# 0x09/dspfun

Measured on AMD Instinct MI355X. Metric: Mpixels/s DCT-II+III roundtrip 3840x2160x3, higher is better.
Workload: dtype f32

## Files before the change

### dspfun_amd/_lib.py

```python
import ctypes as C
import os

_HERE = os.path.dirname(os.path.abspath(__file__))
LIB_PATH = os.environ.get("DSPFFT_LIB_PATH") or os.path.join(_HERE, "csrc", "libdspfft_hip.so")

REDFT01, REDFT10 = 4, 5

SYMBOLS = [
    "dspfft_plan_many_r2r", "dspfft_plan_r2r_2d", "dspfft_plan_set_scale", "dspfft_plan_set_axis_scale0",
    "dspfft_plan_many_r2r_f64", "dspfft_plan_set_scale_f64", "dspfft_plan_set_axis_scale0_f64", "dspfft_execute_f64", "dspfft_execute_masked_accumulate_f64", "dspfft_plan_scan_prepare", "dspfft_plan_set_input_window", "dspfft_plan_set_output_alternate", "dspfft_set_plan_effort", "dspfft_get_plan_effort",
    "dspfft_plan_many_r2r_ordered", "dspfft_plan_guru_r2r", "dspfft_execute_roundtrip", "dspfft_execute_roundtrip_u8", "dspfft_execute_roundtrip_u8_dither",
    "dspfft_roundtrip_topn_work_bytes", "dspfft_execute_roundtrip_topn", "dspfft_execute_roundtrip_u8_topn", "dspfft_motion_topn_blocks_work_bytes", "dspfft_motion_topn_blocks",
    "dspfft_execute", "dspfft_plan_num_passes", "dspfft_execute_pass", "dspfft_destroy_plan", "dspfft_plan_describe", "dspfft_plan_algorithmic_bytes",
    "dspfft_execute_many", "dspfft_execute_many_repeat", "dspfft_execute_sum2", "dspfft_cosrows_create", "dspfft_cosrows_execute", "dspfft_cosrows_destroy", "dspfft_cztrows_create", "dspfft_cztrows_execute", "dspfft_cztrows_execute_n", "dspfft_cztrows_length", "dspfft_cztrows_destroy", "dspfft_transpose_f32", "dspfft_plan_set_input_modulation", "dspfft_stream_create", "dspfft_stream_destroy", "dspfft_stream_synchronize", "dspfft_event_create", "dspfft_event_destroy", "dspfft_event_synchronize", "dspfft_event_elapsed_ms",
    "dspfft_last_error", "dspfft_version", "dspfft_set_thread_plan_effort", "dspfft_get_thread_plan_effort", "dspfft_fftw_sparse_uploads",
    "dspfft_scan_zigzag", "dspfft_scan_zigzag_frame_ids", "dspfft_execute_masked_accumulate", "dspfft_execute_masked_accumulate_range", "dspfft_execute_masked_accumulate_range_f64", "dspfft_scan_scatter", "dspfft_accumulate", "dspfft_broadcast_dc",
    "dspfft_scan_limit", "dspfft_scan_max_interval", "dspfft_scan_coord_slots", "dspfft_scan_owner_index", "dspfft_scan_frame_ids", "dspfft_scan_coords", "dspfft_scan_stamp",
    "dspfft_scan_index_to_frame_ids", "dspfft_scan_magnitude_work_bytes", "dspfft_scan_magnitude_index",
    "dspfft_u8_to_f32", "dspfft_f32_to_u8",
    "dspfft_zoom_ncomponents", "dspfft_zoom_basis", "dspfft_zoom_work_floats", "dspfft_zoom_product", "dspfft_gemm_nt_f32",
    "dspfft_zoom_last_error", "dspfft_zoomfft_create", "dspfft_zoomfft_work_floats", "dspfft_zoomfft_execute", "dspfft_zoomfft_destroy", "dspfft_zoomfft_last_error", "dspfft_zoomczt_create", "dspfft_zoomczt_work_floats", "dspfft_zoomczt_execute", "dspfft_zoomczt_destroy",
    "dspfft_zoomanim_create", "dspfft_zoomanim_work_floats", "dspfft_zoomanim_set_coeffs", "dspfft_zoomanim_execute", "dspfft_zoomanim_destroy", "dspfft_zoomanim_last_error",
    "dspfft_scanframes_create", "dspfft_scanframes_frame_floats", "dspfft_scanframes_begin", "dspfft_scanframes_mark_range", "dspfft_scanframes_mark_coords",
    "dspfft_scanframes_compose", "dspfft_scanframes_parity", "dspfft_scanframes_destroy",
    "dspfft_trc_from_name", "dspfft_trc_name", "dspfft_trc_apply_f32", "dspfft_scanframes_set_trc", "dspfft_zoomanim_set_trc",
    "dspfft_motion_load_f32_linear", "dspfft_motion_store_f32_linear",
    "dspfft_plan_set_u8_trc", "dspfft_u8_to_f32_trc", "dspfft_f32_to_u8_trc", "dspfft_motion_load_u8_linear", "dspfft_motion_store_u8_linear", "dspfft_motion_dither_u8_trc",
    "dspfft_applybasis_work_floats", "dspfft_applybasis_partsums",
    "dspfft_applybasis_work_floats_ex", "dspfft_applybasis_partsums_ex", "dspfft_applybasis_render",
    "dspfft_motion_load_u8", "dspfft_motion_store_u8", "dspfft_motion_load_f32", "dspfft_motion_store_f32", "dspfft_motion_topn_work_bytes", "dspfft_motion_topn", "dspfft_motion_last_error", "dspfft_motion_dither_u8",
    "dspfft_spec_encode", "dspfft_ispec_decode", "dspfft_ispec_signmap", "dspfft_motion_filter", "dspfft_scan_pruned_accumulate", "dspfft_scan_pruned_work_floats", "dspfft_scan_pruned_accumulate_ws", "dspfft_pointwise_last_error",
]

class IoDim(C.Structure):
    _fields_ = [("n", C.c_int), ("is_", C.c_int), ("os", C.c_int)]


class DitherGeom(C.Structure):
    _fields_ = [("n", C.c_int * 3), ("row_pitch", C.c_longlong), ("plane_pitch", C.c_longlong), ("nblocks", C.c_int * 3), ("block_step", C.c_longlong * 3)]


class ScanFrameOpts(C.Structure):
    _fields_ = [("visualize", C.c_int), ("spectrogram", C.c_int), ("intermediates", C.c_int), ("max_intermediates", C.c_int),
                ("spec_gain", C.c_double), ("spec_scaletype", C.c_int), ("spec_signtype", C.c_int), ("parity_depth", C.c_int)]


class MotionFilterParams(C.Structure):
    _fields_ = [("active", C.c_int * 3), ("minbuf_hw", C.c_int * 2), ("block_depth", C.c_int), ("band_begin", C.c_int * 3), ("band_end", C.c_int * 3),
                ("damp", C.c_float), ("boost", C.c_float), ("threshold_lo", C.c_float), ("threshold_hi", C.c_float),
                ("preserve_dc", C.c_int), ("grey_add", C.c_float), ("quantizer", C.c_float)]


_lib = None


def bind(lib):
    ip = C.POINTER(C.c_int)
    vp = C.c_void_p
    lib.dspfft_plan_many_r2r.argtypes = [C.POINTER(vp), C.c_int, ip, C.c_int, ip, C.c_int, C.c_int, ip, C.c_int, C.c_int, ip]
    lib.dspfft_plan_r2r_2d.argtypes = [C.POINTER(vp), C.c_int, C.c_int, C.c_int, C.c_int]
    lib.dspfft_plan_set_scale.argtypes = [vp, C.c_float]
    lib.dspfft_plan_set_axis_scale0.argtypes = [vp, C.c_int, C.c_float, C.c_float]
    lib.dspfft_execute.argtypes = [vp, vp, vp, vp]
    lib.dspfft_execute_sum2.argtypes = [vp, vp, vp, vp, vp, vp]
    lib.dspfft_cosrows_create.argtypes = [C.POINTER(vp), C.c_int, C.c_int, C.c_int, C.c_int]
    lib.dspfft_cosrows_execute.argtypes = [vp, vp, C.c_longlong, vp, C.c_longlong, C.c_double, C.c_double, vp]
    lib.dspfft_cosrows_destroy.argtypes = [vp]
    lib.dspfft_cosrows_destroy.restype = None
    lib.dspfft_cztrows_create.argtypes = [C.POINTER(vp), C.c_int, C.c_int, C.c_int, C.c_int]
    lib.dspfft_cztrows_execute.argtypes = [vp, vp, C.c_longlong, C.c_longlong, C.c_int, vp, C.c_longlong, C.c_longlong, C.c_int, C.c_double, C.c_double, C.c_double, vp]
    lib.dspfft_cztrows_execute_n.argtypes = [vp, C.c_int, C.c_int, vp, C.c_longlong, C.c_longlong, C.c_int, vp, C.c_longlong, C.c_longlong, C.c_int, C.c_double, C.c_double, C.c_double, vp]
    lib.dspfft_zoomanim_create.argtypes = [C.POINTER(vp), C.c_int, C.c_int, C.c_int, C.c_int, C.c_int]
    lib.dspfft_zoomanim_work_floats.restype = C.c_size_t
    lib.dspfft_zoomanim_work_floats.argtypes = [vp]
    lib.dspfft_zoomanim_set_coeffs.argtypes = [vp, vp, vp]
    lib.dspfft_zoomanim_execute.argtypes = [vp] + [C.c_double] * 6 + [C.c_int, C.c_int, vp, vp, vp]
    lib.dspfft_zoomanim_destroy.argtypes = [vp]
    lib.dspfft_zoomanim_destroy.restype = None
    lib.dspfft_zoomanim_last_error.restype = C.c_char_p
    lib.dspfft_cztrows_length.argtypes = [vp]
    lib.dspfft_cztrows_destroy.argtypes = [vp]
    lib.dspfft_cztrows_destroy.restype = None
    lib.dspfft_transpose_f32.argtypes = [vp, C.c_longlong, vp, C.c_longlong, C.c_int, C.c_int, vp]
    lib.dspfft_plan_set_input_modulation.argtypes = [vp, C.c_int, vp, C.c_int]
    lib.dspfft_plan_set_input_window.argtypes = [vp, C.c_int, C.c_int, C.c_int]
    lib.dspfft_plan_set_output_alternate.argtypes = [vp, C.c_int, C.c_int]
    lib.dspfft_execute_many.argtypes = [C.c_int, C.POINTER(vp), C.POINTER(vp), C.POINTER(vp), C.POINTER(vp), C.c_int, C.c_int, C.POINTER(vp)]
    lib.dspfft_execute_many_repeat.argtypes = [C.c_int, C.POINTER(vp), C.POINTER(vp), C.POINTER(vp), C.POINTER(vp), C.c_int, C.c_int, C.c_int, C.c_int, C.POINTER(vp)]
    lib.dspfft_stream_create.restype = vp
    lib.dspfft_stream_create.argtypes = []
    lib.dspfft_stream_destroy.argtypes = [vp]
    lib.dspfft_stream_synchronize.argtypes = [vp]
    lib.dspfft_event_create.restype = vp
    lib.dspfft_event_create.argtypes = []
    lib.dspfft_event_destroy.argtypes = [vp]
    lib.dspfft_event_destroy.restype = None
    lib.dspfft_event_synchronize.argtypes = [vp]
    lib.dspfft_event_elapsed_ms.argtypes = [vp, vp, C.POINTER(C.c_float)]
    lib.dspfft_plan_many_r2r_f64.argtypes = lib.dspfft_plan_many_r2r.argtypes
    lib.dspfft_plan_many_r2r_ordered.argtypes = lib.dspfft_plan_many_r2r.argtypes + [C.c_int]
    lib.dspfft_plan_guru_r2r.argtypes = [C.POINTER(vp), C.c_int, C.POINTER(IoDim), C.c_int, C.POINTER(IoDim), ip, C.c_int]
    lib.dspfft_execute_roundtrip.argtypes = [vp, vp, vp, vp, C.POINTER(MotionFilterParams), vp, vp]
    lib.dspfft_execute_roundtrip_u8.argtypes = [vp, vp, vp, vp, vp, C.c_double, C.POINTER(MotionFilterParams), vp, vp]
    lib.dspfft_execute_roundtrip_u8_dither.argtypes = [vp, vp, vp, vp, vp, C.c_double, C.c_double, C.POINTER(MotionFilterParams), vp, vp]
    if hasattr(lib, "dspfft_execute_roundtrip_topn"):
        lib.dspfft_roundtrip_topn_work_bytes.restype = C.c_size_t
        lib.dspfft_roundtrip_topn_work_bytes.argtypes = [vp, vp]
        lib.dspfft_execute_roundtrip_topn.argtypes = [vp, vp, vp, vp, C.POINTER(MotionFilterParams), C.c_size_t, vp, C.c_size_t, vp, vp]
        lib.dspfft_execute_roundtrip_u8_topn.argtypes = [vp, vp, vp, vp, vp, C.c_double, C.POINTER(MotionFilterParams), C.c_size_t, vp, C.c_size_t, vp, vp]
    lib.dspfft_plan_set_scale_f64.argtypes = [vp, C.c_double]
    lib.dspfft_plan_set_axis_scale0_f64.argtypes = [vp, C.c_int, C.c_double, C.c_double]
    lib.dspfft_execute_f64.argtypes = [vp, vp, vp, vp]
    lib.dspfft_execute_masked_accumulate_f64.argtypes = [vp, vp, vp, vp, vp, C.c_uint32, C.c_int, vp]
    lib.dspfft_plan_scan_prepare.argtypes = [vp, vp, C.c_int, vp]
    lib.dspfft_set_plan_effort.argtypes = [C.c_int]
    lib.dspfft_set_plan_effort.restype = None
    lib.dspfft_get_plan_effort.argtypes = []
    lib.dspfft_plan_num_passes.argtypes = [vp]
    lib.dspfft_execute_pass.argtypes = [vp, C.c_int, vp, vp, vp]
    lib.dspfft_destroy_plan.argtypes = [vp]
    lib.dspfft_destroy_plan.restype = None
    lib.dspfft_plan_describe.argtypes = [vp, C.c_char_p, C.c_size_t]
    lib.dspfft_plan_algorithmic_bytes.argtypes = [vp]
    lib.dspfft_plan_algorithmic_bytes.restype = C.c_size_t
    lib.dspfft_last_error.restype = C.c_char_p
    lib.dspfft_version.restype = C.c_char_p
    lib.dspfft_scan_zigzag.argtypes = [vp, C.c_uint32, C.c_uint32, C.c_uint64, C.c_uint64, vp]
    lib.dspfft_scan_zigzag_frame_ids.argtypes = [vp, C.c_uint32, C.c_uint32, C.c_uint64, vp]
    lib.dspfft_execute_masked_accumulate.argtypes = [vp, vp, vp, vp, vp, C.c_uint32, C.c_int, vp]
    lib.dspfft_execute_masked_accumulate_range.argtypes = [vp, vp, vp, vp, vp, C.c_uint32, C.c_uint32, C.c_int, vp]
    lib.dspfft_execute_masked_accumulate_range_f64.argtypes = [vp, vp, vp, vp, vp, C.c_uint32, C.c_uint32, C.c_int, vp]
    lib.dspfft_scan_limit.restype = C.c_uint64
    lib.dspfft_scan_limit.argtypes = [C.c_int, C.c_uint32, C.c_uint32]
    lib.dspfft_scan_max_interval.restype = C.c_uint64
    lib.dspfft_scan_max_interval.argtypes = [C.c_int, C.c_uint32, C.c_uint32]
    lib.dspfft_scan_coord_slots.restype = C.c_uint64
    lib.dspfft_scan_coord_slots.argtypes = [C.c_int, C.c_uint32, C.c_uint32]
    lib.dspfft_scan_owner_index.argtypes = [vp, C.c_int, C.c_uint32, C.c_uint32, vp]
    lib.dspfft_scan_frame_ids.argtypes = [vp, C.c_int, C.c_uint32, C.c_uint32, C.c_uint64, vp]
    lib.dspfft_scan_coords.argtypes = [vp, C.c_int, C.c_uint32, C.c_uint32, C.c_uint64, C.c_uint64, vp]
    lib.dspfft_scan_stamp.argtypes = [vp, vp, C.c_uint64, C.c_uint32, vp]
# ... 99 lines not shown
```

### dspfun_amd/csrc/dct_spec.h

```cpp
#pragma once
#include "trc_u8_core.h"
#include "dct_core.h"
#include "elementwise_core.h"
#include "spec_list.h"

#ifndef DSP_ROW_PADC
#define DSP_ROW_PADC 1
#endif
#ifndef DSP_COL_PADC
#define DSP_COL_PADC 1
#endif

namespace dspfft {

template <int I, int... Rs> constexpr int pack_get() { constexpr int a[] = {Rs..., 1}; return a[I]; }
template <int I, int... Rs> constexpr int pack_lc() { constexpr int a[] = {Rs..., 1}; int l = 1; for (int j = I; j < (int)sizeof...(Rs); j++) l *= a[j]; return l; }

template <int SPAN, int... Rs> struct PosCalc;
template <int SPAN> struct PosCalc<SPAN> { static DSP_HD int run(int) { return 0; } };
template <int SPAN, int R0, int... Rest>
struct PosCalc<SPAN, R0, Rest...> {
	static DSP_HD int run(int k) { constexpr int span = SPAN / R0; return (k % R0) * span + PosCalc<span, Rest...>::run(k / R0); }
};

// ... 817 lines not shown
		static_for<0, LAST_ROUNDS>([&](auto i) {
			const int it = tid + i * T;
			if (it < NBL * NP) {
				const int kb = it / NP, jp = it - kb * NP;
				int blk;
				if constexpr (NS >= 2) blk = PosCalcFirst<NBL, NS - 1, Rs..., 1>::run(kb); else blk = 0;
				const V *p = buf + (NS >= 2 ? padded(blk * RL) : 0) * NP + jp;
				static_for<0, RL>([&](auto r) { st.x[i * RL + r] = l_get(p[r * NP]); });
				Dft<RL>::run(&st.x[i * RL]);
			}
		});
	}
	template <class ST>
	static DSP_HD void last_write(V *buf, const ST &st, int tid)
	{
		static_for<0, LAST_ROUNDS>([&](auto i) {
			const int it = tid + i * T;
			if (it < NBL * NP) {
				const int kb = it / NP, jp = it - kb * NP;
				V *p = buf + kb * NP + jp;
				static_for<0, RL>([&](auto r) { p[r * NBL * NP] = l_put(st.x[i * RL + r]); });
			}
		});
	}

	static DSP_HD bool lean01(const PA &a) { return !a.accumulate && !a.lean_off; }
	template <int KIND> static DSP_HD bool skip_phase(const PA &a, int ph) { return KIND == KIND_REDFT01 && ph > NS && lean01(a); }
	template <int KIND> static DSP_HD bool barrier_after(const PA &a, int ph) { return (KIND == KIND_REDFT01 && lean01(a)) ? ph < NS : ph + 1 < NPH; }
	static DSP_HD void last_store01(const PA &a, const V *buf, long long bout, int tid)
	{
		static_for<0, LAST_ROUNDS>([&](auto i) {
			const int it = tid + i * T;
			if (it < NBL * NP) {
				const int kb = it / NP, jp = it - kb * NP;
				const V *p = buf + (NS >= 2 ? padded(last_blk(kb) * RL) : 0) * NP + jp;
				LC x[RL];
				static_for<0, RL>([&](auto r) { x[r] = l_get(p[r * NP]); });
				Dft<RL>::run(x);
				static_for<0, RL>([&](auto r) {
					const int y = makhoul_src(kb + NBL * r, N);
					Re sc = (y == 0) ? a.scale * a.out_scale0 : a.scale;
					if (a.alt_out && (y & 1)) sc = -sc;
					*reinterpret_cast<V *>(a.out + bout + (long long)y * a.es_out + VW * jp) = g_put(cmk<LR>(x[r].x * sc, -x[r].y * sc));
				});
			}
		});
	}

	struct StateRT {
		LC x[LAST_ROUNDS * RL];
		LC pre[(Y_ROUNDS > 2 * K_ROUNDS) ? Y_ROUNDS : 2 * K_ROUNDS];
		CX tw[1];
	};
	template <class ST, class F>
	static DSP_HD void mid_read(const PA &af, const PA &ai, const V *buf, long long bout, int tid, ST &st, const F &filt, unsigned long long &coded)
	{
		static_for<0, K_ROUNDS>([&](auto ri) {
			const int it = tid + ri * T;
			if (!((ri + 1) * T <= (N / 2 + 1) * NP || it < (N / 2 + 1) * NP)) return;
			const int k = it / NP, jp = it - k * NP;
			const int km = k ? N - k : 0;
			const LC zk = l_get(buf[k * NP + jp]), zm = l_get(buf[km * NP + jp]);
			const CX t = af.T[k];
			const Re sc = af.scale, s0 = (k == 0) ? sc * af.out_scale0 : sc;
			const long long o = bout + VW * jp;
			LC r0, r1;
			post10(zk, zm, t, s0, sc, r0, r1);
			V xk = g_put(r0), xm = g_put(r1);
			DSP_SCHED_FENCE();
			xk = filt(o + (long long)k * af.es_out, xk, coded);
			DSP_SCHED_FENCE();
			if (k > 0 && km != k) xm = filt(o + (long long)km * af.es_out, xm, coded);
			else if (km == k && k > 0) xm = xk;
			DSP_SCHED_FENCE();
			LC ck = g_get(xk), cm = g_get(xm);
			if (k == 0) { ck = lscale(ck, ai.in_scale0); cm = lzero(); }
			LC lo, hi;
			pre01(ck, cm, t, lo, hi);
			st.pre[2 * ri] = lo; st.pre[2 * ri + 1] = hi;
			DSP_SCHED_FENCE();
		});
	}
	template <class ST>
	static DSP_HD void mid_write(V *buf, int tid, const ST &st)
	{
		static_for<0, K_ROUNDS>([&](auto ri) {
			const int it = tid + ri * T;
			if (!((ri + 1) * T <= (N / 2 + 1) * NP || it < (N / 2 + 1) * NP)) return;
			const int k = it / NP, jp = it - k * NP;
			const int km = k ? N - k : 0;
			buf[padded(k) * NP + jp] = l_put(st.pre[2 * ri]);
			if (k > 0) buf[padded(km) * NP + jp] = l_put(st.pre[2 * ri + 1]);
		});
	}

	template <int KIND, int PH, class ST>
	static DSP_HD void phase(const PA &a, V *buf, long long bout, int tid, ST &st)
	{
		if constexpr (PH == 0) {
			if constexpr (KIND == KIND_REDFT10) {
				static_for<0, Y_ROUNDS>([&](auto i) {
					const int it = tid + i * T;
					if ((i + 1) * T <= N * NP || it < N * NP) {
						const int y = it / NP, jp = it - y * NP;
						LC v = st.pre[i];
						if (y == 0) v = lscale(v, a.in_scale0);
// ... 311 lines not shown
```

### dspfun_amd/csrc/engine.cpp

```cpp
#include <math.h>
#include <stdarg.h>
#include <stdio.h>
#include <stdlib.h>
#include <string.h>

#include <algorithm>
#include <atomic>
#include <complex>
#include <mutex>
#include <dlfcn.h>
#include <memory>
#include <string>
#include <type_traits>
#include <utility>
#include <vector>

#include "../../include/dspfft.h"
#include "backend.h"
#include "scan_frame_core.h"
#include "zoom_anim_core.h"
#include "trc_core.h"
#include "topn_core.h"
#include "block_rt.h"
#include "block_rs_core.h"
// ... 1766 lines not shown
	BlockRtArgs a;
	rt_block_args(c, a);
	if (c.trc_in.id || c.trc_out.id) {
		BlockRtTrcArgs t;
		static_cast<BlockRtArgs &>(t) = a;
		t.keep = (unsigned int)c.keep;
		t.tab_in = (const TrcU8Tab *)c.trc_in.tab; t.tab_out = c.d_out8 ? (const TrcU8Tab *)c.trc_out.tab : nullptr; t.trc_out = c.trc_out.id;
		if (int rc = dspfft_block_trc_launch(&t, c.fwd->blk_nwg, c.fwd->blk_lds, c.stream)) return fail(-4, "kernel launch failed (fused block roundtrip with a transfer characteristic): backend code %d", rc);
		return 0;
	}
	if (c.keep) {
		BlockRtTopnArgs t;
		static_cast<BlockRtArgs &>(t) = a;
		t.keep = (unsigned int)c.keep;
		if (int rc = dspfft_block_topn_launch(&t, c.fwd->blk_nwg, c.fwd->blk_lds, c.stream)) return fail(-4, "kernel launch failed (fused block roundtrip with a coefficient limit): backend code %d", rc);
		return 0;
	}
	if (int rc = be_launch_block_roundtrip(a, c.fwd->blk_nwg, c.fwd->blk_lds, c.stream)) return fail(-4, "kernel launch failed (fused block roundtrip): backend code %d", rc);
	return 0;
}

int rt_topn(const RtCall &c)
{
	if (dspfft_topn_blocks_launch(c.d_out, c.runs.count, c.runs.nblocks, c.runs.stride, c.keep, c.topn_work, c.topn_work_bytes, motion_filter_restores_dc(c.mf), c.stream))
		return fail(-4, "coefficient limit: %s", dspfft_motion_last_error ? dspfft_motion_last_error() : "launch failed");
	return 0;
}

int rt_run_rescale(const RtCall &c)
{
	const dspfft_plan fwd = c.fwd, inv = c.inv;
	const size_t nf = fwd->passes.size(), ni = inv->passes.size();
	float *const d_out = c.d_out;
	if (c.d_in8) {
		if (be_zero(d_out, (size_t)c.span * sizeof(float), c.stream) ||
		    (c.trc_in.id ? dspfft_u8_trc_region_launch(d_out, c.d_in8, c.nf3, c.sw3, c.si3, 0, 1.0, 1.0, 1.0, c.trc_in.id, c.trc_in.tab, c.stream)
		                 : be_region_u8_to_f32(d_out, c.d_in8, c.nf3, c.sw3, c.si3, c.stream))) return fail(-4, "launch failed");
	} else if (c.d_in != d_out) {
		if (be_zero(d_out, (size_t)c.span * sizeof(float), c.stream)) return fail(-4, "launch failed");
	}
	for (size_t i = 0; i < nf; i++) {
		const Pass &P = fwd->passes[i];
		if (int rc = run_pass<float>(fwd, P, (P.first && !c.d_in8) ? c.d_in : d_out, d_out, i + 1 == nf, c.stream)) return rc;
	}
	if (c.keep) if (int rc = rt_topn(c)) return rc;
	if (c.fp && be_motion_filter(d_out, c.mf, (uint64_t)c.span, c.coded, c.stream)) return fail(-4, "filter launch failed");
	for (size_t i = 0; i < ni; i++)
		if (int rc = run_pass<float>(inv, inv->passes[i], (const float *)d_out, d_out, i + 1 == ni, c.stream)) return rc;
	if (c.d_out8 && (c.trc_out.id ? dspfft_u8_trc_region_launch(c.d_out8, d_out, c.ni3, c.sw3, c.sw3, 1, c.mul8, 1.0, 1.0, c.trc_out.id, c.trc_out.tab, c.stream)
	                              : be_region_f32_to_u8(c.d_out8, d_out, c.mul8, c.ni3, c.sw3, c.sw3, c.stream))) return fail(-4, "launch failed");
	return 0;
}

int rt_run_passes(const RtCall &c)
{
	const dspfft_plan fwd = c.fwd, inv = c.inv;
	const size_t nf = fwd->passes.size(), ni = inv->passes.size();
	const Pass &F = *c.F, &I = *c.I;
	float *const d_out = c.d_out;
	void *const stream = c.stream;
	const bool sweep_in = c.d_in8 && !c.u8_first;
	if (sweep_in && rt_u8_in(c, d_out, (uint64_t)c.span)) return fail(-4, "launch failed");
	const float *d_in = sweep_in ? d_out : c.d_in;
	for (size_t i = 0; i + 1 < nf; i++) {
		const Pass &P = fwd->passes[i];
		if (i == 0 && c.d_in8 && c.u8_first) {
			U8IO io; io.in = c.d_in8; io.out = nullptr; io.mul = 1.0;
			if (c.trc_in.id) {
				U8IOTrc t; static_cast<U8IO &>(t) = io; t.tab_in = (const TrcU8Tab *)c.trc_in.tab;
				if (int rc = run_pass_u8_trc(fwd, P, d_out, d_out, false, t, stream)) return rc;
			} else if (int rc = run_pass_u8(fwd, P, d_out, d_out, false, io, stream)) return rc;
			continue;
		}
		if (int rc = run_pass<float>(fwd, P, P.first ? d_in : d_out, d_out, false, stream)) return rc;
	}
	const float *src = nf == 1 ? d_in : d_out;
	const bool listed = F.has_spec && I.has_spec && F.spec.id == I.spec.id;
	const bool compiled = !listed && F.jit && I.jit && F.jit_fn_rt && F.jit_type == I.jit_type;
	const bool fusable = F.type == Pass::COL && I.type == Pass::COL && (listed || compiled) && F.spec_nwg == I.spec_nwg &&
	                     F.hostloop.empty() && I.hostloop.empty() && (15u & ((uintptr_t)src | (uintptr_t)d_out)) == 0 && !fused_roundtrip_off() &&
	                     !c.keep;
	PassArgs af, ai;
	if (fusable) {
		fill_args(af, F.spa, fwd, F, src, d_out, fwd->scale, Fuse());
		fill_args(ai, I.spa, inv, I, (const float *)d_out, d_out, ni == 1 ? inv->scale : 1.0, Fuse());
	}
	if (fusable && is_plain_args(af) && is_plain_args(ai)) {
		if (compiled) {
			void *args[4] = {&af, &ai, (void *)&c.mf, (void *)&c.coded};
			if (int rc = be_jit_launch_n(F.jit_fn_rt, args, F.spec_nwg, F.jit_nthr, stream)) return fail(-4, "kernel launch failed (fused roundtrip, compiled at plan time): backend code %d", rc);
		} else if (int rc = be_launch_roundtrip(F.spec.id, af, ai, c.mf, c.coded, F.spec_nwg, stream)) return fail(-4, "kernel launch failed (fused roundtrip): backend code %d", rc);
	} else {
		if (int rc = run_pass<float>(fwd, F, src, d_out, true, stream)) return rc;
		if (c.keep) if (int rc = rt_topn(c)) return rc;
		if (c.fp && be_motion_filter(d_out, c.mf, (uint64_t)c.span, c.coded, stream)) return fail(-4, "filter launch failed");
		if (int rc = run_pass<float>(inv, I, (const float *)d_out, d_out, ni == 1, stream)) return rc;
	}
	for (size_t i = 1; i < ni; i++) {
		const Pass &P = inv->passes[i];
		if (i + 1 == ni && c.d_out8 && c.u8_last) {
			U8IO io; io.in = nullptr; io.out = c.d_out8; io.mul = c.mul8;
			if (c.trc_out.id) {
				U8IOTrc t; static_cast<U8IO &>(t) = io; t.tab_out = (const TrcU8Tab *)c.trc_out.tab; t.trc_out = c.trc_out.id;
				if (int rc = run_pass_u8_trc(inv, P, d_out, d_out, true, t, stream)) return rc;
			} else if (int rc = run_pass_u8(inv, P, d_out, d_out, true, io, stream)) return rc;
			continue;
		}
		if (int rc = run_pass<float>(inv, P, (const float *)d_out, d_out, i + 1 == ni, stream)) return rc;
	}
	if (c.d_out8 && !c.u8_last && rt_u8_out(c, d_out, (uint64_t)c.span)) return fail(-4, "launch failed");
	return 0;
}

constexpr size_t kSliceBytes = 100u << 20;
constexpr int kSliceTileK = 8;

struct SliceSwitches { int forced, nstreams; };
const SliceSwitches &slice_switches()
{
	static const SliceSwitches s = []() {
		const char *f = getenv("DSPFFT_RT_SLICE"), *n = getenv("DSPFFT_RT_STREAMS");
		return SliceSwitches{f ? atoi(f) : -1, std::min(2, std::max(1, n ? atoi(n) : 2))};
	}();
	return s;
}

int slice_frames(const dspfft_plan_s *fwd, const dspfft_plan_s *inv, const dspfft_motion_filter_params *fp)
{
	const int forced = slice_switches().forced, nstreams = slice_switches().nstreams;
	if (forced == 0 || fwd->rank != 2 || fwd->batches.size() != 1 || inv->batches.size() != 1 || fwd->passes.size() != 2 || inv->passes.size() != 2) return 0;
	if (fwd->col_kpref || inv->col_kpref) return 0;
	const Pass &F = fwd->passes[1], &I = inv->passes[0];
	if (F.type != Pass::COL || I.type != Pass::COL || !F.has_spec || !I.has_spec || F.jit || I.jit) return 0;
	SpecInfo narrow;
	if (!be_find_spec(1, F.pa.N, F.pa.ninner, &narrow, kSliceTileK) || narrow.P != kSliceTileK || narrow.P == F.spec.P) return 0;
	const Dim &b = fwd->batches[0];
	const long long frame = b.os;
	if (frame <= 0 || inv->batches[0].is != b.os || inv->batches[0].os != b.os) return 0;
	long long S = forced > 0 ? forced : (long long)(kSliceBytes * (nstreams > 1 ? 1 : 2) / ((size_t)frame * sizeof(float)));
	if (forced <= 0 && b.n < 4 * S) S = (b.n + 3) / 4;
// ... 151 lines not shown
	if (!(scalefactor > 0) || !(normalization > 0)) return fail(-1, "dither: scalefactor and normalization must be > 0");
	dspfft_dither_geom g;
	if (int rc = dither_geom_of(inv, g)) return rc;
	const Dither dz = {d_out, scalefactor, normalization};
	return roundtrip_core(fwd, inv, nullptr, d_work, d_in, nullptr, 1.0, fp, d_coeffs_coded, stream, true, &dz);
}

extern "C" int dspfft_scan_zigzag_frame_ids(uint32_t *d_ids, uint32_t w, uint32_t h, uint64_t step, void *s)
{
	if (!d_ids || !w || !h || !step) return fail(-1, "bad arguments");
	if ((uint64_t)w * h > 0xffffffffull) return fail(-1, "image too large for 32-bit offsets");
	return be_scan_zigzag_frame_ids(d_ids, w, h, step, s) ? fail(-4, "launch failed") : 0;
}

extern "C" int dspfft_plan_num_passes(dspfft_plan pl) { return pl ? (int)pl->passes.size() : 0; }

extern "C" int dspfft_execute_pass(dspfft_plan pl, int index, const float *d_in, float *d_out, void *stream)
{
	if (!pl || !d_in || !d_out || index < 0 || index >= (int)pl->passes.size()) return fail(-1, "bad plan, buffer or pass index");
	if (pl->f64) return fail(-1, "dspfft_execute_pass takes f32 plans");
	const std::vector<Pass> &passes = pick_passes(pl, d_in, d_out);
	const Pass &P = passes[index];
	return run_pass<float>(pl, P, P.first ? d_in : d_out, d_out, index + 1 == (int)passes.size(), stream);
}

template <class R>
static int execute_item(dspfft_plan pl, const void *in, void *out, void *st, bool timed, void *const *pass_events, int &ev)
{
	const R *d_in = (const R *)in;
	R *d_out = (R *)out;
	if (!timed) return execute_t<R>(pl, d_in, d_out, st);
	const std::vector<Pass> &passes = pick_passes(pl, d_in, d_out);
	for (size_t p = 0; p < passes.size(); p++) {
		const Pass &P = passes[p];
		if (be_event_record(pass_events[ev++], st)) return fail(-4, "event record failed");
		if (int rc = run_pass<R>(pl, P, P.first ? d_in : d_out, d_out, p + 1 == passes.size(), st)) return rc;
		if (be_event_record(pass_events[ev++], st)) return fail(-4, "event record failed");
	}
	return 0;
}
struct ChanLinesGuard {
	bool on = false;
	ChanLinesGuard(int count, const dspfft_plan *plans, void *const *streams)
	{
		void *first = nullptr; bool have = false;
		for (int i = 0; streams && i < count && !on; i++) {
			if (!plans[i] || !plans[i]->f64) continue;
			if (!have) { first = streams[i]; have = true; } else if (streams[i] != first) on = true;
		}
		if (on) g_chan_lines_suspended++;
	}
	~ChanLinesGuard() { if (on) g_chan_lines_suspended--; }
};
static int execute_many_once(int count, const dspfft_plan *plans, const void *const *d_in, void *const *d_out, void *const *streams,
                             int timed_item, int timed_count, void *const *pass_events)
{
	ChanLinesGuard guard(count, plans, streams);
	int ev = 0;
	for (int i = 0; i < count; i++) {
		dspfft_plan pl = plans[i];
		void *st = streams ? streams[i] : nullptr;
		const bool timed = pass_events && i >= timed_item && i < timed_item + timed_count;
		const int rc = pl->f64 ? execute_item<double>(pl, d_in[i], d_out[i], st, timed, pass_events, ev) : execute_item<float>(pl, d_in[i], d_out[i], st, timed, pass_events, ev);
		if (rc) return rc;
	}
	return 0;
}
static bool plan_is_staged(const dspfft_plan_s *pl)
{
	for (const Pass &P : pl->passes) if (P.tab.stage) return true;
	return false;
}
static int check_many(int count, const dspfft_plan *plans, const void *const *d_in, void *const *d_out, void *const *streams, int timed_item, int timed_count, bool events, bool f64_ok)
{
	if (count < 0 || (count && (!plans || !d_in || !d_out))) return fail(-1, "bad arguments");
	for (int i = 0; i < count; i++) {
		if (!plans[i] || !d_in[i] || !d_out[i]) return fail(-1, "item %d: null plan or buffer", i);
		if (plans[i]->f64 && !f64_ok) return fail(-1, "dspfft_execute_many takes f32 plans");
		if (streams && plan_is_staged(plans[i]))
			for (int j = 0; j < i; j++)
				if (plans[j] == plans[i] && streams[j] != streams[i]) return fail(-1, "items %d and %d: a plan with a staged pass (its lines pass through a device array of the plan) cannot run on two streams at once", j, i);
	}
	if (events) {
		if (timed_item < 0 || timed_count < 0 || timed_item + timed_count > count) return fail(-1, "timed items [%d, %d) lie outside the batch of %d", timed_item, timed_item + timed_count, count);
		for (int i = timed_item; i < timed_item + timed_count; i++)
			if (plans[i]->has_block) return fail(-1, "item %d: per-pass events are not available for one-pass block plans", i);
	}
	return 0;
}

extern "C" int dspfft_execute_many(int count, const dspfft_plan *plans, const float *const *d_in, float *const *d_out, void *const *streams,
                                   int timed_item, int timed_count, void *const *pass_events)
{
	if (int rc = check_many(count, plans, (const void *const *)d_in, (void *const *)d_out, streams, timed_item, timed_count, pass_events != nullptr, false)) return rc;
	return execute_many_once(count, plans, (const void *const *)d_in, (void *const *)d_out, streams, timed_item, timed_count, pass_events);
}

extern "C" int dspfft_execute_many_repeat(int count, const dspfft_plan *plans, const void *const *d_in, void *const *d_out, void *const *streams,
                                          int repeats, int rejoin_every, int timed_every, int timed_count, void *const *pass_events)
{
	if (repeats < 0 || rejoin_every < 0 || timed_every < 0) return fail(-1, "bad arguments");
	const bool ev = pass_events && timed_every > 0 && timed_count > 0;
	if (ev && count % timed_count) return fail(-1, "the timed window (%d items) must divide the batch (%d items)", timed_count, count);
	if (int rc = check_many(count, plans, d_in, d_out, streams, 0, ev ? count : 0, ev, true)) return rc;
	std::vector<void *> uniq;
	for (int i = 0; i < count; i++) { void *st = streams ? streams[i] : nullptr; if (std::find(uniq.begin(), uniq.end(), st) == uniq.end()) uniq.push_back(st); }
	std::vector<void *> join;
	const bool rejoin = rejoin_every > 0 && uniq.size() > 1;
	if (rejoin) for (size_t i = 0; i < uniq.size(); i++) { void *e = be_order_event_create(); if (!e) { for (void *x : join) be_event_destroy(x); return fail(-4, "event creation failed"); } join.push_back(e); }
	int rc = 0, windows = 0;
	size_t ev_off = 0;
	for (int k = 0; k < repeats && !rc; k++) {
		if (rejoin && k && k % rejoin_every == 0) {
			for (size_t a = 0; a < uniq.size() && !rc; a++) if (be_event_record(join[a], uniq[a])) rc = fail(-4, "event record failed");
			for (size_t a = 0; a < uniq.size() && !rc; a++)
				for (size_t b = 0; b < uniq.size() && !rc; b++)
					if (a != b && be_stream_wait_event(uniq[a], join[b])) rc = fail(-4, "stream wait failed");
			if (rc) break;
		}
		if (ev && k % timed_every == 0) {
			const int first = (int)(((long long)windows * timed_count) % count);
			rc = execute_many_once(count, plans, d_in, d_out, streams, first, timed_count, pass_events + ev_off);
			for (int i = first; i < first + timed_count; i++) ev_off += 2 * pick_passes(plans[i], d_in[i], d_out[i]).size();
			windows++;
		} else rc = execute_many_once(count, plans, d_in, d_out, streams, 0, 0, nullptr);
	}
	for (void *x : join) be_event_destroy(x);
	return rc;
}
extern "C" void *dspfft_stream_create(void) { return be_stream_create(); }
extern "C" void dspfft_stream_destroy(void *s) { be_stream_destroy(s); }
extern "C" int dspfft_stream_synchronize(void *s) { return be_stream_synchronize(s) ? fail(-4, "stream synchronise failed") : 0; }
extern "C" void *dspfft_event_create(void) { return be_event_create(); }
extern "C" void dspfft_event_destroy(void *e) { be_event_destroy(e); }
extern "C" int dspfft_event_synchronize(void *e) { return e && !be_event_synchronize(e) ? 0 : fail(-4, "event synchronise failed"); }
extern "C" int dspfft_event_elapsed_ms(void *a, void *b, float *ms)
{
	if (!a || !b || !ms) return fail(-1, "bad arguments");
	return be_event_elapsed_ms(a, b, ms) ? fail(-4, "event query failed") : 0;
}

extern "C" void dspfft_destroy_plan(dspfft_plan pl)
{
	if (!pl) return;
	for (Pass &P : pl->passes) P.tab.release();
	for (Pass &P : pl->split) P.tab.release();
	be_free(pl->zflags); be_free(pl->zpage); be_free(pl->zranges); be_free(pl->eids);
	if (pl->u8_tab_owned) be_free(pl->u8_tab);
	delete pl;
}

extern "C" int dspfft_plan_describe(dspfft_plan pl, char *buf, size_t buflen)
{
	if (!pl || !buf || !buflen) return fail(-1, "bad arguments");
	std::string s = std::string("backend ") + be_name() + "\n";
	for (const Pass &P : pl->split) { s += P.desc; s += "\n"; }
	if (pl->has_block) { s += pl->blk_desc; s += "\n"; }
	for (const Pass &P : pl->passes) { if (!pl->split.empty() || pl->has_block) s += "plain "; s += P.desc; if (!P.hostloop.empty()) s += " +hostloop"; s += "\n"; }
	if (pl->u8_trc) { s += "8-bit end of a roundtrip through transfer characteristic "; s += trc_name(pl->u8_trc); s += "\n"; }
	std::lock_guard<std::mutex> lock(pl->rt_mutex);
	for (const auto &r : pl->rt_slices) {
		char b[256];
		snprintf(b, sizeof b, "roundtrip_u8 in slices of %d frames (last: %d) on %d stream(s): ", r->frames, r->fwd_rem ? r->fwd_rem->howmany : r->frames, r->side ? 2 : 1);
		s += b; s += r->fwd->passes.back().desc; s += "\n";
	}
	snprintf(buf, buflen, "%s", s.c_str());
	return 0;
}

extern "C" size_t dspfft_plan_algorithmic_bytes(dspfft_plan pl) { return pl ? pl->alg_bytes : 0; }
#undef g_plan_effort
extern "C" void dspfft_set_plan_effort(int effort) { g_plan_effort_default.store(effort < 0 ? 0 : effort, std::memory_order_relaxed); }
extern "C" int dspfft_get_plan_effort(void) { return t_plan_effort >= 0 ? t_plan_effort : g_plan_effort_default.load(std::memory_order_relaxed); }
extern "C" void dspfft_set_thread_plan_effort(int effort) { t_plan_effort = effort < 0 ? -1 : effort; }
extern "C" int dspfft_get_thread_plan_effort(void) { return t_plan_effort; }

extern "C" int dspfft_scan_zigzag(uint32_t *d_lin, uint32_t w, uint32_t h, uint64_t first, uint64_t count, void *s)
{
// ... 354 lines not shown
```

### dspfun_amd/csrc/spec_fused.h

```cpp
#pragma once
#include <hip/hip_runtime.h>
#include "dct_spec.h"
#ifndef DSP_STAMP
#define DSP_STAMP(i) ((void)0)
#endif
#include "motion_filter.h"

namespace dspfft {

struct FilterOp {
	MotionFilter p;
	__device__ SigVec<float, 2> operator()(long long e, SigVec<float, 2> v, unsigned long long &coded) const
	{
		if (!p.enabled) return v;
		float4 f; f.x = v.s[0].x; f.y = v.s[0].y; f.z = v.s[1].x; f.w = v.s[1].y;
		f = motion_filter4(p, (uint32_t)e, f, coded);
		v.s[0].x = f.x; v.s[0].y = f.y; v.s[1].x = f.z; v.s[1].y = f.w;
		return v;
	}
};

template <class S> constexpr int rt_waves_per_simd()
{
	const int wgs = (int)((160 * 1024) / S::LDS), w = wgs * S::T / 256;
	return w < 1 ? 1 : w > 4 ? 4 : w;
}

template <class PA> __host__ __device__ inline PA plain_args(const PA &a_)
{
	PA a = a_;
	a.mask = nullptr; a.zflags = nullptr; a.zranges = nullptr; a.accumulate = 0; a.win_lo = a.win_hi = 0; a.alt_out = 0; a.in_mul = nullptr; a.in_rev = 0;
	return a;
}
template <class PA> static inline bool is_plain(const PA &a) { return !a.mask && !a.zflags && !a.accumulate && a.win_hi <= 0 && !a.alt_out && !a.in_mul && !a.in_rev; }

template <class S>
__device__ __forceinline__ void col_roundtrip_body(unsigned char *lds, const typename S::PA &af_, const typename S::PA &ai_, const FilterOp &filt, unsigned long long *coded)
{
	const typename S::PA af = plain_args(af_), ai = plain_args(ai_);
	__shared__ unsigned int wg_coded;
	typename S::V *buf = reinterpret_cast<typename S::V *>(lds);
	const int tid = threadIdx.x;
	if (tid == 0) wg_coded = 0;
	typename S::StateRT st;
	long long bin, bout;
	S::base(af, blockIdx.x, bin, bout);
	bool hit = false;
	DSP_STAMP(0);
	S::template prefetch<KIND_REDFT10>(af, bin, tid, st, hit);
	S::template phase<KIND_REDFT10, 0>(af, buf, bout, tid, st);
	__syncthreads();
	DSP_STAMP(1);
	static_for<1, S::NS + 2>([&](auto ph) {
		int t = tid; asm volatile("" : "+v"(t));
		S::template phase<KIND_REDFT10, ph>(af, buf, bout, t, st);
		__syncthreads();
		DSP_STAMP(1 + ph);
	});
	unsigned long long mine = 0;
	int t = tid; asm volatile("" : "+v"(t));
	S::mid_read(af, ai, buf, bout, t, st, filt, mine);
	if (coded) {
		unsigned int m = (unsigned int)mine;
		for (int off = 32; off > 0; off >>= 1) m += __shfl_xor(m, off);
		if ((tid & 63) == 0 && m) atomicAdd(&wg_coded, m);
	}
	__syncthreads();
	DSP_STAMP(10);
	if (coded && tid == 0 && wg_coded) atomicAdd(coded, (unsigned long long)wg_coded);
	asm volatile("" : "+v"(t));
	S::mid_write(buf, t, st);
	__syncthreads();
	DSP_STAMP(11);
	typename S::PA a2 = ai;
	asm volatile("" : "+s"(a2.W), "+s"(a2.T), "+s"(a2.out));
	static_for<1, S::NPH>([&](auto ph) {
		asm volatile("" : "+v"(t));
		S::template phase<KIND_REDFT01, ph>(a2, buf, bout, t, st);
		if constexpr (ph + 1 < S::NPH) __syncthreads();
		DSP_STAMP(12 + ph);
	});
}

}
```

### dspfun_amd/engine.py

```python
import ctypes as C

from . import _lib

REDFT01, REDFT10 = _lib.REDFT01, _lib.REDFT10


class DspfftError(RuntimeError):
    pass


def _ia(v):
    return None if v is None else (C.c_int * len(v))(*[int(x) for x in v])


def set_plan_effort(effort, lib=None):
    (lib or _lib.load()).dspfft_set_plan_effort(int(effort))


class Plan:

    def __init__(self, handle, lib, f64=False):
        self._h = handle
        self._lib = lib
        self.f64 = f64
# ... 422 lines not shown

def _ptr(t):
    if t is None:
        return None
    return C.c_void_p(t if isinstance(t, int) else t.data_ptr())


def scan_frame_rgb(frame, w, h, visualize=False, intermediates=False):
    fw, fh = w * (1 + bool(visualize)), h * (1 + bool(intermediates))
    return frame.reshape(3, fh, fw)[[2, 0, 1]]


class Stream:

    def __init__(self, lib=None):
        self._lib = lib or _lib.load()
        self.handle = self._lib.dspfft_stream_create()
        if not self.handle:
            raise DspfftError("stream creation failed")

    def synchronize(self):
        if self._lib.dspfft_stream_synchronize(self.handle):
            raise DspfftError(self._lib.dspfft_last_error().decode())

    def __del__(self):
        try:
            self._lib.dspfft_stream_destroy(self.handle)
        except Exception:
            pass


class Events:

    def __init__(self, n, lib=None):
        self._lib = lib or _lib.load()
        self.handles = (C.c_void_p * n)(*[self._lib.dspfft_event_create() for _ in range(n)])
        if any(h is None for h in self.handles):
            raise DspfftError("event creation failed")

    def elapsed_ms(self, i, j):
        ms = C.c_float()
        if self._lib.dspfft_event_elapsed_ms(self.handles[i], self.handles[j], C.byref(ms)):
            raise DspfftError(self._lib.dspfft_last_error().decode())
        return float(ms.value)

    def __del__(self):
        try:
            for h in self.handles:
                self._lib.dspfft_event_destroy(h)
        except Exception:
            pass


class Batch:

    def __init__(self, items, lib=None):
        items = list(items)
        self._lib = lib or _lib.load()
        self._keep = [it[0] for it in items]
        n = len(items)
        self.n = n
        self._plans = (C.c_void_p * n)(*[it[0]._h for it in items])
        self._in = (C.c_void_p * n)(*[it[1] for it in items])
        self._out = (C.c_void_p * n)(*[(it[1] if it[2] is None else it[2]) for it in items])
        self._streams = (C.c_void_p * n)(*[(it[3] or None) for it in items])

    def run(self, timed_item=0, timed_count=0, events=None, event_offset=0):
        ev = None
        if events is not None and timed_count:
            ev = C.cast(C.byref(events.handles, event_offset * C.sizeof(C.c_void_p)), C.POINTER(C.c_void_p))
        rc = self._lib.dspfft_execute_many(self.n, self._plans, self._in, self._out, self._streams, timed_item, timed_count if ev is not None else 0, ev)
        if rc:
            raise DspfftError(self._lib.dspfft_last_error().decode())

    def run_repeat(self, repeats, rejoin_every=0, timed_every=0, timed_count=0, events=None):
        ev = None
        if events is not None and timed_every and timed_count:
            ev = C.cast(events.handles, C.POINTER(C.c_void_p))
        rc = self._lib.dspfft_execute_many_repeat(self.n, self._plans, self._in, self._out, self._streams, int(repeats), int(rejoin_every),
                                                  int(timed_every) if ev is not None else 0, int(timed_count) if ev is not None else 0, ev)
        if rc:
            raise DspfftError(self._lib.dspfft_last_error().decode())
```

### include/dspfft.h

```cpp
#ifndef DSPFFT_H
#define DSPFFT_H
#include <stddef.h>
#include <stdint.h>
#ifdef __cplusplus
extern "C" {
#endif

enum { DSPFFT_REDFT01 = 4, DSPFFT_REDFT10 = 5 };

typedef struct dspfft_plan_s *dspfft_plan;

int dspfft_plan_many_r2r(dspfft_plan *plan, int rank, const int *n, int howmany,
                         const int *inembed, int istride, int idist,
                         const int *onembed, int ostride, int odist, const int *kinds);

int dspfft_plan_r2r_2d(dspfft_plan *plan, int n0, int n1, int kind0, int kind1);

int dspfft_plan_set_scale(dspfft_plan plan, float scale);
int dspfft_plan_set_axis_scale0(dspfft_plan plan, int axis, float in_scale0, float out_scale0);

int dspfft_execute(dspfft_plan plan, const float *d_in, float *d_out, void *hip_stream);

int dspfft_plan_num_passes(dspfft_plan plan);
int dspfft_execute_pass(dspfft_plan plan, int index, const float *d_in, float *d_out, void *hip_stream);

int dspfft_execute_many(int count, const dspfft_plan *plans, const float *const *d_in, float *const *d_out, void *const *hip_streams,
                        int timed_item, int timed_count, void *const *pass_events);
int dspfft_execute_many_repeat(int count, const dspfft_plan *plans, const void *const *d_in, void *const *d_out, void *const *hip_streams,
                               int repeats, int rejoin_every, int timed_every, int timed_count, void *const *pass_events);
void *dspfft_stream_create(void);
void dspfft_stream_destroy(void *stream);
int dspfft_stream_synchronize(void *stream);
void *dspfft_event_create(void);
void dspfft_event_destroy(void *event);
int dspfft_event_synchronize(void *event);
int dspfft_event_elapsed_ms(void *start, void *stop, float *ms);

int dspfft_plan_many_r2r_f64(dspfft_plan *plan, int rank, const int *n, int howmany,
                             const int *inembed, int istride, int idist,
                             const int *onembed, int ostride, int odist, const int *kinds);
int dspfft_plan_set_scale_f64(dspfft_plan plan, double scale);
int dspfft_plan_set_axis_scale0_f64(dspfft_plan plan, int axis, double in_scale0, double out_scale0);
int dspfft_execute_f64(dspfft_plan plan, const double *d_in, double *d_out, void *hip_stream);
int dspfft_plan_set_input_window(dspfft_plan plan, int axis, int lo, int hi);
int dspfft_plan_set_input_modulation(dspfft_plan plan, int axis, const float *d_mul, int reversed_from);
int dspfft_plan_set_output_alternate(dspfft_plan plan, int axis, int on);
int dspfft_execute_sum2(dspfft_plan a, dspfft_plan b, const float *d_in_a, const float *d_in_b, float *d_out, void *hip_stream);

typedef struct dspfft_cosrows_s *dspfft_cosrows;
int dspfft_cosrows_create(dspfft_cosrows *plan, int M, int cw, int vw, int lines);
int dspfft_cosrows_execute(dspfft_cosrows plan, const float *d_in, long long in_pitch, float *d_out, long long out_pitch, double theta, double scale, void *hip_stream);
void dspfft_cosrows_destroy(dspfft_cosrows plan);

typedef struct dspfft_cztrows_s *dspfft_cztrows;
int dspfft_cztrows_create(dspfft_cztrows *plan, int nc, int nout, int lines, int group);
int dspfft_cztrows_execute(dspfft_cztrows plan, const float *d_in, long long in_group, long long in_pitch, int es_in,
                           float *d_out, long long out_group, long long out_pitch, int es_out, double omega, double phi, double scale, void *hip_stream);
int dspfft_cztrows_execute_n(dspfft_cztrows plan, int nc, int lines, const float *d_in, long long in_group, long long in_pitch, int es_in,
                             float *d_out, long long out_group, long long out_pitch, int es_out, double omega, double phi, double scale, void *hip_stream);
int dspfft_cztrows_length(dspfft_cztrows plan);
void dspfft_cztrows_destroy(dspfft_cztrows plan);
int dspfft_transpose_f32(float *d_out, long long out_pitch, const float *d_in, long long in_pitch, int rows, int cols, void *hip_stream);
int dspfft_plan_scan_prepare(dspfft_plan plan, const uint32_t *d_ids, int elems_per_id, void *hip_stream);
int dspfft_execute_masked_accumulate_f64(dspfft_plan plan, const double *d_in, double *d_work, double *d_acc,
                                         const uint32_t *d_ids, uint32_t id, int elems_per_id, void *hip_stream);

typedef struct { int n; int is; int os; } dspfft_iodim;
void dspfft_set_plan_effort(int effort);
int dspfft_get_plan_effort(void);
void dspfft_set_thread_plan_effort(int effort);
int dspfft_get_thread_plan_effort(void);
unsigned long long dspfft_fftw_sparse_uploads(void);
int dspfft_plan_guru_r2r(dspfft_plan *plan, int rank, const dspfft_iodim *dims, int howmany_rank, const dspfft_iodim *howmany_dims,
                         const int *kinds, int f64);

int dspfft_plan_many_r2r_ordered(dspfft_plan *plan, int rank, const int *n, int howmany,
                                 const int *inembed, int istride, int idist,
                                 const int *onembed, int ostride, int odist, const int *kinds, int first_axis_first);

typedef struct {
	int active[3];
	int minbuf_hw[2];
// ... 206 lines not shown
```

Before: 61170.

## Fuse adjacent forward/inverse DCT plan pairs in execute_many into roundtrip kernel

execute_many and execute_many_repeat now look for consecutive plan pairs (forward then inverse, same stream, in-place chaining) that qualify for the fused column roundtrip kernel, and launch a single fused roundtrip for each such pair instead of two separate executions. This is meant to remove an extra kernel launch and a global-memory round trip of the intermediate spectrum. The fused kernel also scopes its per-phase register state into separate blocks (forward state, mid state, inverse state) to shorten live ranges and lower register pressure. A counter is exported for observability. Timed items are excluded from fusion.

```diff
diff --git a/dspfun_amd/_lib.py b/dspfun_amd/_lib.py
--- a/dspfun_amd/_lib.py
+++ b/dspfun_amd/_lib.py
@@ -12,7 +12,7 @@
     "dspfft_plan_many_r2r_ordered", "dspfft_plan_guru_r2r", "dspfft_execute_roundtrip", "dspfft_execute_roundtrip_u8", "dspfft_execute_roundtrip_u8_dither",
     "dspfft_roundtrip_topn_work_bytes", "dspfft_execute_roundtrip_topn", "dspfft_execute_roundtrip_u8_topn", "dspfft_motion_topn_blocks_work_bytes", "dspfft_motion_topn_blocks",
     "dspfft_execute", "dspfft_plan_num_passes", "dspfft_execute_pass", "dspfft_destroy_plan", "dspfft_plan_describe", "dspfft_plan_algorithmic_bytes",
-    "dspfft_execute_many", "dspfft_execute_many_repeat", "dspfft_execute_sum2", "dspfft_cosrows_create", "dspfft_cosrows_execute", "dspfft_cosrows_destroy", "dspfft_cztrows_create", "dspfft_cztrows_execute", "dspfft_cztrows_execute_n", "dspfft_cztrows_length", "dspfft_cztrows_destroy", "dspfft_transpose_f32", "dspfft_plan_set_input_modulation", "dspfft_stream_create", "dspfft_stream_destroy", "dspfft_stream_synchronize", "dspfft_event_create", "dspfft_event_destroy", "dspfft_event_synchronize", "dspfft_event_elapsed_ms",
+    "dspfft_execute_many", "dspfft_execute_many_repeat", "dspfft_many_fused_pairs", "dspfft_execute_sum2", "dspfft_cosrows_create", "dspfft_cosrows_execute", "dspfft_cosrows_destroy", "dspfft_cztrows_create", "dspfft_cztrows_execute", "dspfft_cztrows_execute_n", "dspfft_cztrows_length", "dspfft_cztrows_destroy", "dspfft_transpose_f32", "dspfft_plan_set_input_modulation", "dspfft_stream_create", "dspfft_stream_destroy", "dspfft_stream_synchronize", "dspfft_event_create", "dspfft_event_destroy", "dspfft_event_synchronize", "dspfft_event_elapsed_ms",
     "dspfft_last_error", "dspfft_version", "dspfft_set_thread_plan_effort", "dspfft_get_thread_plan_effort", "dspfft_fftw_sparse_uploads",
     "dspfft_scan_zigzag", "dspfft_scan_zigzag_frame_ids", "dspfft_execute_masked_accumulate", "dspfft_execute_masked_accumulate_range", "dspfft_execute_masked_accumulate_range_f64", "dspfft_scan_scatter", "dspfft_accumulate", "dspfft_broadcast_dc",
     "dspfft_scan_limit", "dspfft_scan_max_interval", "dspfft_scan_coord_slots", "dspfft_scan_owner_index", "dspfft_scan_frame_ids", "dspfft_scan_coords", "dspfft_scan_stamp",
@@ -87,6 +87,9 @@
     lib.dspfft_plan_set_output_alternate.argtypes = [vp, C.c_int, C.c_int]
     lib.dspfft_execute_many.argtypes = [C.c_int, C.POINTER(vp), C.POINTER(vp), C.POINTER(vp), C.POINTER(vp), C.c_int, C.c_int, C.POINTER(vp)]
     lib.dspfft_execute_many_repeat.argtypes = [C.c_int, C.POINTER(vp), C.POINTER(vp), C.POINTER(vp), C.POINTER(vp), C.c_int, C.c_int, C.c_int, C.c_int, C.POINTER(vp)]
+    if hasattr(lib, "dspfft_many_fused_pairs"):
+        lib.dspfft_many_fused_pairs.restype = C.c_ulonglong
+        lib.dspfft_many_fused_pairs.argtypes = []
     lib.dspfft_stream_create.restype = vp
     lib.dspfft_stream_create.argtypes = []
     lib.dspfft_stream_destroy.argtypes = [vp]
diff --git a/dspfun_amd/csrc/dct_spec.h b/dspfun_amd/csrc/dct_spec.h
--- a/dspfun_amd/csrc/dct_spec.h
+++ b/dspfun_amd/csrc/dct_spec.h
@@ -893,6 +893,7 @@
 		LC pre[(Y_ROUNDS > 2 * K_ROUNDS) ? Y_ROUNDS : 2 * K_ROUNDS];
 		CX tw[1];
 	};
+	struct StateMid { LC pre[2 * K_ROUNDS]; };
 	template <class ST, class F>
 	static DSP_HD void mid_read(const PA &af, const PA &ai, const V *buf, long long bout, int tid, ST &st, const F &filt, unsigned long long &coded)
 	{
diff --git a/dspfun_amd/csrc/engine.cpp b/dspfun_amd/csrc/engine.cpp
--- a/dspfun_amd/csrc/engine.cpp
+++ b/dspfun_amd/csrc/engine.cpp
@@ -1842,6 +1842,21 @@
 	return 0;
 }
 
+bool rt_col_fused(const RtCall &c, const float *src, PassArgs &af, PassArgs &ai, bool &compiled)
+{
+	const dspfft_plan fwd = c.fwd, inv = c.inv;
+	const Pass &F = *c.F, &I = *c.I;
+	const bool listed = F.has_spec && I.has_spec && F.spec.id == I.spec.id;
+	compiled = !listed && F.jit && I.jit && F.jit_fn_rt && F.jit_type == I.jit_type;
+	const bool fusable = F.type == Pass::COL && I.type == Pass::COL && (listed || compiled) && F.spec_nwg == I.spec_nwg &&
+	                     F.hostloop.empty() && I.hostloop.empty() && (15u & ((uintptr_t)src | (uintptr_t)c.d_out)) == 0 && !fused_roundtrip_off() &&
+	                     !c.keep;
+	if (!fusable) return false;
+	fill_args(af, F.spa, fwd, F, src, c.d_out, fwd->scale, Fuse());
+	fill_args(ai, I.spa, inv, I, (const float *)c.d_out, c.d_out, inv->passes.size() == 1 ? inv->scale : 1.0, Fuse());
+	return is_plain_args(af) && is_plain_args(ai);
+}
+
 int rt_run_passes(const RtCall &c)
 {
 	const dspfft_plan fwd = c.fwd, inv = c.inv;
@@ -1865,17 +1880,9 @@
 		if (int rc = run_pass<float>(fwd, P, P.first ? d_in : d_out, d_out, false, stream)) return rc;
 	}
 	const float *src = nf == 1 ? d_in : d_out;
-	const bool listed = F.has_spec && I.has_spec && F.spec.id == I.spec.id;
-	const bool compiled = !listed && F.jit && I.jit && F.jit_fn_rt && F.jit_type == I.jit_type;
-	const bool fusable = F.type == Pass::COL && I.type == Pass::COL && (listed || compiled) && F.spec_nwg == I.spec_nwg &&
-	                     F.hostloop.empty() && I.hostloop.empty() && (15u & ((uintptr_t)src | (uintptr_t)d_out)) == 0 && !fused_roundtrip_off() &&
-	                     !c.keep;
 	PassArgs af, ai;
-	if (fusable) {
-		fill_args(af, F.spa, fwd, F, src, d_out, fwd->scale, Fuse());
-		fill_args(ai, I.spa, inv, I, (const float *)d_out, d_out, ni == 1 ? inv->scale : 1.0, Fuse());
-	}
-	if (fusable && is_plain_args(af) && is_plain_args(ai)) {
+	bool compiled;
+	if (rt_col_fused(c, src, af, ai, compiled)) {
 		if (compiled) {
 			void *args[4] = {&af, &ai, (void *)&c.mf, (void *)&c.coded};
 			if (int rc = be_jit_launch_n(F.jit_fn_rt, args, F.spec_nwg, F.jit_nthr, stream)) return fail(-4, "kernel launch failed (fused roundtrip, compiled at plan time): backend code %d", rc);
@@ -2133,8 +2140,42 @@
 	}
 	~ChanLinesGuard() { if (on) g_chan_lines_suspended--; }
 };
+static std::atomic<unsigned long long> g_many_fused_pairs{0};
+extern "C" unsigned long long dspfft_many_fused_pairs(void) { return g_many_fused_pairs.load(std::memory_order_relaxed); }
+
+struct ManyPairs { std::vector<RtCall> calls; };
+static bool many_pair_check(const dspfft_plan *plans, const void *const *d_in, void *const *d_out, void *const *streams, int i, RtCall &c)
+{
+	const dspfft_plan fwd = plans[i], inv = plans[i + 1];
+	if (fwd->f64 || inv->f64 || (streams && streams[i] != streams[i + 1]) || d_out[i] != d_in[i + 1] || d_in[i + 1] != d_out[i + 1]) return false;
+	if (fwd->has_block || inv->has_block || &pick_passes(fwd, d_in[i], d_out[i]) != &fwd->passes || &pick_passes(inv, d_in[i + 1], d_out[i + 1]) != &inv->passes) return false;
+	if (fwd->passes.empty() || inv->passes.empty()) return false;
+	c = RtCall{fwd, inv, (const float *)d_in[i], (float *)d_out[i], nullptr, nullptr, 1.0, nullptr, nullptr, streams ? streams[i] : nullptr, 0, nullptr, 0};
+	char err[sizeof g_err];
+	memcpy(err, g_err, sizeof err);
+	const bool ok = rt_check(c) == 0 && !c.grid && !c.block && !c.rescale;
+	memcpy(g_err, err, sizeof err);
+	if (!ok) return false;
+	PassArgs af, ai;
+	bool compiled;
+	return rt_col_fused(c, fwd->passes.size() == 1 ? c.d_in : c.d_out, af, ai, compiled);
+}
+static void many_pairs_find(int count, const dspfft_plan *plans, const void *const *d_in, void *const *d_out, void *const *streams, ManyPairs &mp)
+{
+	mp.calls.clear();
+	if (count < 2 || fused_roundtrip_off()) return;
+	mp.calls.resize((size_t)count);
+	bool any = false;
+	for (int i = 0; i + 1 < count; i++) {
+		RtCall c;
+		if (many_pair_check(plans, d_in, d_out, streams, i, c)) { mp.calls[i] = c; any = true; } else mp.calls[i].fwd = nullptr;
+	}
+	mp.calls[count - 1].fwd = nullptr;
+	if (!any) mp.calls.clear();
+}
+
 static int execute_many_once(int count, const dspfft_plan *plans, const void *const *d_in, void *const *d_out, void *const *streams,
-                             int timed_item, int timed_count, void *const *pass_events)
+                             int timed_item, int timed_count, void *const *pass_events, const ManyPairs &mp)
 {
 	ChanLinesGuard guard(count, plans, streams);
 	int ev = 0;
@@ -2142,6 +2183,12 @@
 		dspfft_plan pl = plans[i];
 		void *st = streams ? streams[i] : nullptr;
 		const bool timed = pass_events && i >= timed_item && i < timed_item + timed_count;
+		if (!mp.calls.empty() && mp.calls[i].fwd && !timed && !(pass_events && i + 1 >= timed_item && i + 1 < timed_item + timed_count)) {
+			if (int rc = rt_run_passes(mp.calls[i])) return rc;
+			g_many_fused_pairs.fetch_add(1, std::memory_order_relaxed);
+			i++;
+			continue;
+		}
 		const int rc = pl->f64 ? execute_item<double>(pl, d_in[i], d_out[i], st, timed, pass_events, ev) : execute_item<float>(pl, d_in[i], d_out[i], st, timed, pass_events, ev);
 		if (rc) return rc;
 	}
@@ -2174,7 +2221,9 @@
                                    int timed_item, int timed_count, void *const *pass_events)
 {
 	if (int rc = check_many(count, plans, (const void *const *)d_in, (void *const *)d_out, streams, timed_item, timed_count, pass_events != nullptr, false)) return rc;
-	return execute_many_once(count, plans, (const void *const *)d_in, (void *const *)d_out, streams, timed_item, timed_count, pass_events);
+	ManyPairs mp;
+	many_pairs_find(count, plans, (const void *const *)d_in, (void *const *)d_out, streams, mp);
+	return execute_many_once(count, plans, (const void *const *)d_in, (void *const *)d_out, streams, timed_item, timed_count, pass_events, mp);
 }
 
 extern "C" int dspfft_execute_many_repeat(int count, const dspfft_plan *plans, const void *const *d_in, void *const *d_out, void *const *streams,
@@ -2189,6 +2238,8 @@
 	std::vector<void *> join;
 	const bool rejoin = rejoin_every > 0 && uniq.size() > 1;
 	if (rejoin) for (size_t i = 0; i < uniq.size(); i++) { void *e = be_order_event_create(); if (!e) { for (void *x : join) be_event_destroy(x); return fail(-4, "event creation failed"); } join.push_back(e); }
+	ManyPairs mp;
+	if (repeats > 0) many_pairs_find(count, plans, d_in, d_out, streams, mp);
 	int rc = 0, windows = 0;
 	size_t ev_off = 0;
 	for (int k = 0; k < repeats && !rc; k++) {
@@ -2201,10 +2252,10 @@
 		}
 		if (ev && k % timed_every == 0) {
 			const int first = (int)(((long long)windows * timed_count) % count);
-			rc = execute_many_once(count, plans, d_in, d_out, streams, first, timed_count, pass_events + ev_off);
+			rc = execute_many_once(count, plans, d_in, d_out, streams, first, timed_count, pass_events + ev_off, mp);
 			for (int i = first; i < first + timed_count; i++) ev_off += 2 * pick_passes(plans[i], d_in[i], d_out[i]).size();
 			windows++;
-		} else rc = execute_many_once(count, plans, d_in, d_out, streams, 0, 0, nullptr);
+		} else rc = execute_many_once(count, plans, d_in, d_out, streams, 0, 0, nullptr, mp);
 	}
 	for (void *x : join) be_event_destroy(x);
 	return rc;
diff --git a/dspfun_amd/csrc/spec_fused.h b/dspfun_amd/csrc/spec_fused.h
--- a/dspfun_amd/csrc/spec_fused.h
+++ b/dspfun_amd/csrc/spec_fused.h
@@ -42,38 +42,44 @@
 	typename S::V *buf = reinterpret_cast<typename S::V *>(lds);
 	const int tid = threadIdx.x;
 	if (tid == 0) wg_coded = 0;
-	typename S::StateRT st;
 	long long bin, bout;
 	S::base(af, blockIdx.x, bin, bout);
 	bool hit = false;
 	DSP_STAMP(0);
-	S::template prefetch<KIND_REDFT10>(af, bin, tid, st, hit);
-	S::template phase<KIND_REDFT10, 0>(af, buf, bout, tid, st);
-	__syncthreads();
-	DSP_STAMP(1);
-	static_for<1, S::NS + 2>([&](auto ph) {
-		int t = tid; asm volatile("" : "+v"(t));
-		S::template phase<KIND_REDFT10, ph>(af, buf, bout, t, st);
+	{
+		typename S::template State<KIND_REDFT10> st;
+		S::template prefetch<KIND_REDFT10>(af, bin, tid, st, hit);
+		S::template phase<KIND_REDFT10, 0>(af, buf, bout, tid, st);
 		__syncthreads();
-		DSP_STAMP(1 + ph);
-	});
-	unsigned long long mine = 0;
+		DSP_STAMP(1);
+		static_for<1, S::NS + 2>([&](auto ph) {
+			int t = tid; asm volatile("" : "+v"(t));
+			S::template phase<KIND_REDFT10, ph>(af, buf, bout, t, st);
+			__syncthreads();
+			DSP_STAMP(1 + ph);
+		});
+	}
 	int t = tid; asm volatile("" : "+v"(t));
-	S::mid_read(af, ai, buf, bout, t, st, filt, mine);
-	if (coded) {
-		unsigned int m = (unsigned int)mine;
-		for (int off = 32; off > 0; off >>= 1) m += __shfl_xor(m, off);
-		if ((tid & 63) == 0 && m) atomicAdd(&wg_coded, m);
+	{
+		typename S::StateMid st;
+		unsigned long long mine = 0;
+		S::mid_read(af, ai, buf, bout, t, st, filt, mine);
+		if (coded) {
+			unsigned int m = (unsigned int)mine;
+			for (int off = 32; off > 0; off >>= 1) m += __shfl_xor(m, off);
+			if ((tid & 63) == 0 && m) atomicAdd(&wg_coded, m);
+		}
+		__syncthreads();
+		DSP_STAMP(10);
+		if (coded && tid == 0 && wg_coded) atomicAdd(coded, (unsigned long long)wg_coded);
+		asm volatile("" : "+v"(t));
+		S::mid_write(buf, t, st);
+		__syncthreads();
+		DSP_STAMP(11);
 	}
-	__syncthreads();
-	DSP_STAMP(10);
-	if (coded && tid == 0 && wg_coded) atomicAdd(coded, (unsigned long long)wg_coded);
-	asm volatile("" : "+v"(t));
-	S::mid_write(buf, t, st);
-	__syncthreads();
-	DSP_STAMP(11);
 	typename S::PA a2 = ai;
 	asm volatile("" : "+s"(a2.W), "+s"(a2.T), "+s"(a2.out));
+	typename S::template State<KIND_REDFT01> st;
 	static_for<1, S::NPH>([&](auto ph) {
 		asm volatile("" : "+v"(t));
 		S::template phase<KIND_REDFT01, ph>(a2, buf, bout, t, st);
diff --git a/dspfun_amd/engine.py b/dspfun_amd/engine.py
--- a/dspfun_amd/engine.py
+++ b/dspfun_amd/engine.py
@@ -498,6 +498,10 @@
             pass
 
 
+def many_fused_pairs(lib=None):
+    return int((lib or _lib.load()).dspfft_many_fused_pairs())
+
+
 class Batch:
 
     def __init__(self, items, lib=None):
diff --git a/include/dspfft.h b/include/dspfft.h
--- a/include/dspfft.h
+++ b/include/dspfft.h
@@ -28,6 +28,7 @@
                         int timed_item, int timed_count, void *const *pass_events);
 int dspfft_execute_many_repeat(int count, const dspfft_plan *plans, const void *const *d_in, void *const *d_out, void *const *hip_streams,
                                int repeats, int rejoin_every, int timed_every, int timed_count, void *const *pass_events);
+unsigned long long dspfft_many_fused_pairs(void);
 void *dspfft_stream_create(void);
 void dspfft_stream_destroy(void *stream);
 int dspfft_stream_synchronize(void *stream);
```

After: 67480, median of 6. 10.3% higher.
